# ChainSafe/Spectre

Hardware: NVIDIA H100
Metric: bn254_g1_msm_pairs_per_s (higher is better)
Workload: dtype u256 (8x32-bit Montgomery limbs, INT32 IMAD)

## Files before the change

spectre_b200/csrc/msm.cu:

```cuda
#define SPB_MSM_KERNELS 1
#include "common.cuh"
#include "msm.cuh"
#include <cub/device/device_scan.cuh>
#include <string.h>

using namespace spb;

struct SrsShard {
  int dev_index = 0;
  size_t start = 0, count = 0;
  G1Affine* g = nullptr;
  G1Affine* g_lagrange = nullptr;
};
struct spb_srs {
  uint32_t k = 0;
  size_t n = 0;
  unsigned char g2[128] = {0}, s_g2[128] = {0};
  uint32_t table_c = 0;
  std::vector<SrsShard> shards;
};


namespace spb {

typedef MsmLane Lane;
static const size_t kLanePinnedBytes = 256 * 1024;
static int get_lane(spb_ctx* ctx, int dev_index, int lane_index, Lane** out) {
  Lane& l = ctx->dev[dev_index].lanes[lane_index];
  if (!l.ready) {
    SPB_CUDA(ctx, cudaStreamCreateWithFlags(&l.stream, cudaStreamNonBlocking));
    for (int i = 0; i < 9; i++) SPB_CUDA(ctx, cudaEventCreate(&l.ev[i]));
    SPB_CUDA(ctx, cudaMallocHost(&l.pinned, kLanePinnedBytes));
    l.ready = true;
  }
  *out = &l;
  return 0;
}

void msm_release_ctx(spb_ctx* ctx) {
  for (auto& d : ctx->dev) {
    cudaSetDevice(d.device);
    for (auto& l : d.lanes) {
      if (!l.ready) continue;
      cudaStreamSynchronize(l.stream);
      for (int i = 0; i < 9; i++) cudaEventDestroy(l.ev[i]);
      cudaFreeHost(l.pinned);
      cudaStreamDestroy(l.stream);
      l = Lane();
    }
  }
}

static void* lane_slot(spb_ctx* ctx, DeviceState& d, int lane, const char* name, size_t bytes) {
  char buf[64];
  snprintf(buf, sizeof buf, "%s#%d", name, lane);
  return slot(ctx, d, buf, bytes);
}

static uint32_t choose_chunk(const DeviceState& d, uint64_t est_entries) {
  const double wave = (double)d.sm_count * 512.0;
  if (est_entries >= kLongChunkMinEntries) return kLongChunk;
  double waves = (double)est_entries / 32.0 / wave;
  if (waves < 1.0) return 32;
  double w = waves < 1.5 ? 1.0 : (double)(uint64_t)(waves + 0.5);
  uint32_t L = (uint32_t)((double)est_entries / (w * wave)) + 1;
  if (L < 24) L = 24;
  if (L > 48) L = 48;
  return L;
}

static int msm_enqueue(spb_ctx* ctx, DeviceState& d, int lane, Lane& ln, const Fr* d_scalars, const G1Affine* d_bases, uint64_t n, MsmGeom g) {
  const uint64_t nb = (uint64_t)g.BW * g.B;
  const uint64_t cap = n * g.W;
  const uint32_t Lmin = g.L == kLongChunk ? kShortChunk : g.L;
  const uint64_t Tmax = (cap + Lmin - 1) / Lmin;
  if (cap >= 0x7fffffffull) return set_error(ctx, SPB_ERR_ARG, "msm: %llu entries exceed the 31-bit sort index", (unsigned long long)cap);
  uint32_t* counts = (uint32_t*)lane_slot(ctx, d, lane, "msm_counts", (nb + 1) * 4);
  uint32_t* offsets = (uint32_t*)lane_slot(ctx, d, lane, "msm_offsets", (nb + 1) * 4);
  MsmEntry* ent = (MsmEntry*)lane_slot(ctx, d, lane, "msm_entries", (cap + 1) * sizeof(MsmEntry));
  G1Xyzz* buckets = (G1Xyzz*)lane_slot(ctx, d, lane, "msm_buckets", nb * sizeof(G1Xyzz));
  uint32_t* head_key = (uint32_t*)lane_slot(ctx, d, lane, "msm_head_key", (Tmax + 1) * 4);
  uint32_t* tail_key = (uint32_t*)lane_slot(ctx, d, lane, "msm_tail_key", (Tmax + 1) * 4);
  G1Xyzz* head = (G1Xyzz*)lane_slot(ctx, d, lane, "msm_head", (Tmax + 1) * sizeof(G1Xyzz));
  G1Xyzz* tail = (G1Xyzz*)lane_slot(ctx, d, lane, "msm_tail", (Tmax + 1) * sizeof(G1Xyzz));
  uint32_t* giant = (uint32_t*)lane_slot(ctx, d, lane, "msm_giant", (Tmax + 2) * 4);
  const uint64_t max_huge = Tmax / kHugeChain + 1;
  uint32_t* huge = (uint32_t*)lane_slot(ctx, d, lane, "msm_huge", (2 * max_huge + 2) * 4);
  G1Xyzz* huge_part = (G1Xyzz*)lane_slot(ctx, d, lane, "msm_huge_part", max_huge * kHugeBlocks * sizeof(G1Xyzz));
  const MsmTail tl = msm_tail_shape(g.c);
  const uint32_t R = 1u << tl.r_log, C = 1u << tl.c_log, per = msm_tail_partials(tl);
  const uint32_t T1 = g.B >> tl.m_log;
  const uint64_t ngroups = (uint64_t)g.BW * T1;
  G1Xyzz* grp = (G1Xyzz*)lane_slot(ctx, d, lane, "msm_groups", 2 * ngroups * sizeof(G1Xyzz));
  G1Xyzz* seg_out = (G1Xyzz*)lane_slot(ctx, d, lane, "msm_rowcol", (uint64_t)g.BW * (2 * R + C) * sizeof(G1Xyzz));
  G1Xyzz* win_out = (G1Xyzz*)lane_slot(ctx, d, lane, "msm_partials", (uint64_t)g.BW * per * sizeof(G1Xyzz));
  size_t scan_bytes = 0;
  cub::DeviceScan::ExclusiveSum(nullptr, scan_bytes, counts, offsets, (int)(nb + 1), ln.stream);
  void* scan_tmp = lane_slot(ctx, d, lane, "msm_scan_tmp", scan_bytes ? scan_bytes : 16);
  if (!counts || !offsets || !ent || !buckets || !head_key || !tail_key || !head || !tail || !giant || !huge || !huge_part || !grp || !seg_out || !win_out || !scan_tmp)
    return SPB_ERR_OOM;
  if ((size_t)g.BW * per * sizeof(G1Xyzz) + 16 > kLanePinnedBytes) return set_error(ctx, SPB_ERR_STATE, "msm: %u window partials exceed the pinned staging area", g.BW * per);

  cudaStream_t st = ln.stream;
  SPB_CUDA(ctx, cudaMemsetAsync(giant, 0, 4, st));
  SPB_CUDA(ctx, cudaMemsetAsync(huge, 0, 4, st));
  const unsigned tb = 256;
  SPB_CUDA(ctx, cudaMemsetAsync(counts, 0, (nb + 1) * 4, st));
  cudaEventRecord(ln.ev[0], st);
  msm_count_kernel<<<(unsigned)((n + tb - 1) / tb), tb, 0, st>>>(n, d_scalars, g, counts);
  cudaEventRecord(ln.ev[1], st);
  SPB_CUDA(ctx, cub::DeviceScan::ExclusiveSum(scan_tmp, scan_bytes, counts, offsets, (int)(nb + 1), st));
  SPB_CUDA(ctx, cudaMemcpyAsync(counts, offsets, (nb + 1) * 4, cudaMemcpyDeviceToDevice, st));
  cudaEventRecord(ln.ev[2], st);
  msm_scatter_kernel<<<(unsigned)((n + tb - 1) / tb), tb, 0, st>>>(n, d_scalars, g, counts, ent);
  const uint32_t* total = offsets + nb;
  cudaEventRecord(ln.ev[3], st);
  msm_accumulate_kernel<<<(unsigned)((Tmax + 127) / 128), 128, 0, st>>>(total, g, ent, d_bases, buckets, head_key, head, tail_key, tail);
  cudaEventRecord(ln.ev[4], st);
  msm_stitch_kernel<<<(unsigned)((Tmax + 127) / 128), 128, 0, st>>>(total, g.L, 24, head_key, head, tail_key, tail, buckets, giant, giant + 1);
  msm_giant_kernel<<<256, 128, 0, st>>>(total, g.L, giant, giant + 1, head_key, head, tail_key, tail, buckets, huge, huge + 2);
  msm_huge_kernel<<<kHugeBlocks, 128, 0, st>>>(huge, huge + 2, head, huge_part);
  msm_huge_finish_kernel<<<64, 128, 0, st>>>(huge, huge + 2, kHugeBlocks, huge_part, tail_key, tail, buckets);
  cudaEventRecord(ln.ev[5], st);
  G1Xyzz *rows = seg_out, *cols = seg_out + (uint64_t)g.BW * R, *wrows = seg_out + (uint64_t)g.BW * (R + C);
  msm_group_kernel<<<(unsigned)((ngroups + 127) / 128), 128, 0, st>>>(ngroups, tl.m_log, offsets, buckets, grp, grp + ngroups);
  cudaEventRecord(ln.ev[6], st);
  msm_rowcol_kernel<<<g.BW * (2 * R + C), 64, 0, st>>>(T1, tl, grp, grp + ngroups, rows, cols, wrows);
  msm_weighted_kernel<<<g.BW * (2 * tl.nbr + tl.nbc), 128, 0, st>>>(tl, rows, cols, wrows, win_out);
  cudaEventRecord(ln.ev[7], st);
  SPB_CUDA(ctx, cudaGetLastError());
  ctx->n_kernel_launches += 10;
  SPB_CUDA(ctx, cudaMemcpyAsync(ln.pinned, win_out, (size_t)g.BW * per * sizeof(G1Xyzz), cudaMemcpyDeviceToHost, st));
  SPB_CUDA(ctx, cudaMemcpyAsync((char*)ln.pinned + (size_t)g.BW * per * sizeof(G1Xyzz), total, 4, cudaMemcpyDeviceToHost, st));
  return 0;
}

static G1Xyzz msm_finish(Lane& ln, MsmGeom g, uint64_t* adds) {
  const MsmTail tl = msm_tail_shape(g.c);
  const uint32_t per = msm_tail_partials(tl);
  const G1Xyzz* P = (const G1Xyzz*)ln.pinned;
  uint32_t M; memcpy(&M, (const char*)ln.pinned + (size_t)g.BW * per * sizeof(G1Xyzz), 4);
  if (adds) *adds += (uint64_t)M + 2ull * g.BW * g.B;
  std::vector<G1Xyzz> S(g.BW);
  for (uint32_t w = 0; w < g.BW; w++) S[w] = msm_tail_finish(g, P + (size_t)w * per);
  return msm_combine_windows(S.data(), g.BW, g.c);
}

static void write_result(const G1Xyzz& r, spb_g1* out) {
  G1Affine a = xyzz_to_affine(r);
  G1Jac j = jac_from_affine(a);
  memcpy(out, &j, sizeof(G1Jac));
}

struct MsmPart {
  int dev_index;
  const Fr* d_scalars;
  const Fr* h_scalars;
  int peer_src_device;
  const G1Affine* d_bases;
  uint64_t n;
  MsmGeom g;
};

static int job_enqueue(spb_ctx* ctx, int lane, std::vector<MsmPart>& parts) {
  for (auto& p : parts) {
    if (!p.n) continue;
    DeviceState& d = ctx->dev[p.dev_index];
    SPB_CUDA(ctx, cudaSetDevice(d.device));
    Lane* ln; SPB_TRY(get_lane(ctx, p.dev_index, lane, &ln));
    p.g.L = choose_chunk(d, p.n * p.g.W);
    const Fr* ds = p.d_scalars;
    DeviceState& src = p.peer_src_device >= 0 ? ctx->dev[0] : d;
    if (&src != &d) SPB_CUDA(ctx, cudaSetDevice(src.device));
    SPB_CUDA(ctx, cudaEventRecord(src.dep_ev, src.stream));
    if (&src != &d) SPB_CUDA(ctx, cudaSetDevice(d.device));
    SPB_CUDA(ctx, cudaStreamWaitEvent(ln->stream, src.dep_ev, 0));
    SPB_CUDA(ctx, cudaEventRecord(ln->ev[8], ln->stream));
    if (p.h_scalars || p.peer_src_device >= 0) {
      Fr* buf = (Fr*)lane_slot(ctx, d, lane, "msm_scalars", p.n * sizeof(Fr));
      if (!buf) return SPB_ERR_OOM;
      if (p.h_scalars) SPB_CUDA(ctx, cudaMemcpyAsync(buf, p.h_scalars, p.n * sizeof(Fr), cudaMemcpyHostToDevice, ln->stream));
      else SPB_CUDA(ctx, cudaMemcpyPeerAsync(buf, d.device, p.d_scalars, p.peer_src_device, p.n * sizeof(Fr), ln->stream));
      ds = buf;
    }
    SPB_TRY(msm_enqueue(ctx, d, lane, *ln, ds, p.d_bases, p.n, p.g));
  }
  return 0;
}

static int job_collect(spb_ctx* ctx, int lane, const std::vector<MsmPart>& parts, spb_g1* out) {
  G1Xyzz acc = xyzz_identity();
  float worst = 0.f;
  for (auto& p : parts) {
    if (!p.n) continue;
    DeviceState& d = ctx->dev[p.dev_index];
    SPB_CUDA(ctx, cudaSetDevice(d.device));
    Lane* ln; SPB_TRY(get_lane(ctx, p.dev_index, lane, &ln));
    SPB_CUDA(ctx, cudaStreamSynchronize(ln->stream));
    float ms = 0.f;
    SPB_CUDA(ctx, cudaEventElapsedTime(&ms, ln->ev[8], ln->ev[7]));
    if (ms > worst) worst = ms;
    if (p.dev_index == 0) for (int e = 0; e < 7; e++) cudaEventElapsedTime(&ctx->msm_stage_ms[e], ln->ev[e], ln->ev[e + 1]);
    G1Xyzz r = msm_finish(*ln, p.g, &ctx->last_msm_adds);
// ... 484 lines not shown
```

spectre_b200/csrc/msm.cuh:

```cuda
#pragma once
#include <stdlib.h>
#include "curve.cuh"

namespace spb {

struct MsmGeom {
  uint32_t c;
  uint32_t W;
  uint32_t B;
  uint32_t L;
  uint32_t BW;
  uint32_t precomp;
  uint32_t tab_stride;
};

struct alignas(8) MsmEntry { uint32_t key, val; };

static const uint32_t kLongChunk = 96, kShortChunk = 32;
#ifndef SPB_LONG_CHUNK_MIN_ENTRIES
#define SPB_LONG_CHUNK_MIN_ENTRIES (1ull << 23)
#endif
static const uint64_t kLongChunkMinEntries = SPB_LONG_CHUNK_MIN_ENTRIES;
SPB_HD uint32_t msm_effective_chunk(uint32_t L, uint64_t M) { return (L == kLongChunk && M < kLongChunkMinEntries) ? kShortChunk : L; }

static const uint32_t kNoKey = 0xffffffffu;

#if defined(__CUDA_ARCH__)
SPB_D uint32_t spb_atomic_inc(uint32_t* p) { return atomicAdd(p, 1u); }
#else
inline uint32_t spb_atomic_inc(uint32_t* p) { uint32_t v = *p; *p = v + 1; return v; }
#endif

struct DigitIter {
  uint32_t limbs[8];
  uint32_t c, carry, w;
  SPB_HD void init(const Fr& canonical, uint32_t c_) {
    for (int i = 0; i < 8; i++) limbs[i] = canonical.l[i];
    c = c_; carry = 0; w = 0;
  }
  SPB_HD int32_t next() {
    uint32_t bit = w * c, word = bit >> 5, sh = bit & 31;
    uint64_t v = 0;
    if (word < 8) {
      v = limbs[word];
      if (word + 1 < 8) v |= (uint64_t)limbs[word + 1] << 32;
      v >>= sh;
    }
    uint32_t raw = (uint32_t)(v & ((1u << c) - 1)) + carry;
    w++;
    if (raw > (1u << (c - 1))) { carry = 1; return (int32_t)raw - (int32_t)(1u << c); }
    carry = 0;
    return (int32_t)raw;
  }
};

SPB_HD void msm_count_thread(uint64_t tid, uint64_t n, const Fr* scalars, MsmGeom g, uint32_t* counts) {
  if (tid >= n) return;
  Fr s = fp_from_mont(scalars[tid]);
  if (fp_is_zero(s)) return;
  DigitIter it; it.init(s, g.c);
  for (uint32_t w = 0; w < g.W; w++) {
    int32_t d = it.next();
    if (d == 0) continue;
    uint32_t mag = d < 0 ? (uint32_t)(-d) : (uint32_t)d;
    spb_atomic_inc(&counts[(g.precomp ? 0u : w * g.B) + mag - 1]);
  }
}

SPB_HD void msm_scatter_thread(uint64_t tid, uint64_t n, const Fr* scalars, MsmGeom g, uint32_t* cursor, MsmEntry* ent) {
  if (tid >= n) return;
  Fr s = fp_from_mont(scalars[tid]);
  if (fp_is_zero(s)) return;
  DigitIter it; it.init(s, g.c);
  for (uint32_t w = 0; w < g.W; w++) {
    int32_t d = it.next();
    if (d == 0) continue;
    uint32_t mag = d < 0 ? (uint32_t)(-d) : (uint32_t)d;
    uint32_t key = (g.precomp ? 0u : w * g.B) + mag - 1;
    uint32_t pos = spb_atomic_inc(&cursor[key]);
    MsmEntry e; e.key = key; e.val = ((uint32_t)tid + (g.precomp ? w * g.tab_stride : 0u)) | (d < 0 ? 0x80000000u : 0u);
    ent[pos] = e;
  }
}

SPB_HD G1Affine msm_load_point(const G1Affine* bases, uint32_t val) {
#if defined(__CUDA_ARCH__)
  const uint4* q = reinterpret_cast<const uint4*>(bases + (val & 0x7fffffffu));
  uint4 a = __ldg(q), b = __ldg(q + 1), c = __ldg(q + 2), d = __ldg(q + 3);
  G1Affine p;
  p.x.l[0] = a.x; p.x.l[1] = a.y; p.x.l[2] = a.z; p.x.l[3] = a.w; p.x.l[4] = b.x; p.x.l[5] = b.y; p.x.l[6] = b.z; p.x.l[7] = b.w;
  p.y.l[0] = c.x; p.y.l[1] = c.y; p.y.l[2] = c.z; p.y.l[3] = c.w; p.y.l[4] = d.x; p.y.l[5] = d.y; p.y.l[6] = d.z; p.y.l[7] = d.w;
#else
  G1Affine p = bases[val & 0x7fffffffu];
#endif
  if (val & 0x80000000u) p.y = fp_neg(p.y);
  return p;
}

SPB_HD MsmEntry msm_load_entry(const MsmEntry* p) {
#if defined(__CUDA_ARCH__)
  uint2 v = __ldg(reinterpret_cast<const uint2*>(p));
  MsmEntry e; e.key = v.x; e.val = v.y; return e;
#else
  return *p;
#endif
}

SPB_HD void msm_accumulate_thread(uint64_t tid, uint64_t M, MsmGeom g, const MsmEntry* ent,
                                  const G1Affine* bases, G1Xyzz* buckets, uint32_t* head_key, G1Xyzz* head,
                                  uint32_t* tail_key, G1Xyzz* tail) {
  const uint32_t L = msm_effective_chunk(g.L, M);
  uint64_t lo = tid * L;
  if (lo >= M) return;
  uint64_t hi = lo + L < M ? lo + L : M;
  uint32_t hk = kNoKey, tk = kNoKey;
  MsmEntry first = msm_load_entry(ent + lo);
  uint32_t cur = first.key;
  bool run_started_before = lo > 0 && msm_load_entry(ent + lo - 1).key == cur;
  G1Xyzz acc = xyzz_from_affine(msm_load_point(bases, first.val));
  for (uint64_t e = lo + 1; e < hi; e++) {
    MsmEntry en = msm_load_entry(ent + e);
    uint32_t k = en.key;
    G1Affine p = msm_load_point(bases, en.val);
    if (k == cur) {
      xyzz_add_mixed(acc, p);
    } else {
      if (run_started_before) { hk = cur; head[tid] = acc; }
      else buckets[cur] = acc;
      run_started_before = false;
      cur = k;
      acc = xyzz_from_affine(p);
    }
  }
  bool continues = hi < M && msm_load_entry(ent + hi).key == cur;
  if (continues) {
    if (run_started_before) { hk = cur; head[tid] = acc; }
    else { tk = cur; tail[tid] = acc; }
  } else {
    if (run_started_before) { hk = cur; head[tid] = acc; }
    else buckets[cur] = acc;
  }
  head_key[tid] = hk;
  tail_key[tid] = tk;
}

SPB_HD void msm_stitch_thread(uint64_t tid, uint64_t T, uint32_t cap, const uint32_t* head_key, const G1Xyzz* head,
                              const uint32_t* tail_key, const G1Xyzz* tail, G1Xyzz* buckets, uint32_t* giant_count,
                              uint32_t* giant_list) {
  if (tid >= T) return;
  uint32_t key = tail_key[tid];
  if (key == kNoKey) return;
  uint64_t j = tid + 1, len = 0;
  while (j < T && head_key[j] == key && len <= cap) { j++; len++; }
  if (len > cap) { uint32_t slot = spb_atomic_inc(giant_count); giant_list[slot] = (uint32_t)tid; return; }
  G1Xyzz acc = tail[tid];
  for (uint64_t q = tid + 1; q < tid + 1 + len; q++) xyzz_add(acc, head[q]);
  buckets[key] = acc;
}

struct MsmTail {
  uint32_t m_log;
  uint32_t r_log, c_log;
  uint32_t nbr, nbc;
};
inline MsmTail msm_tail_shape(uint32_t c) {
  MsmTail t; uint32_t bits = c - 1;
  t.m_log = bits < 3 ? bits : 3;
  bits -= t.m_log;
  t.c_log = bits / 2; t.r_log = bits - t.c_log;
  t.nbr = ((1u << t.r_log) + 127) / 128; t.nbc = ((1u << t.c_log) + 127) / 128;
  return t;
}
SPB_HD uint32_t msm_tail_partials(const MsmTail& t) { return 3 * t.nbr + 2 * t.nbc; }

SPB_HD void msm_group_thread(uint64_t tid, uint64_t ngroups, uint32_t m_log, const uint32_t* offsets, const G1Xyzz* buckets, G1Xyzz* s1, G1Xyzz* w1) {
  if (tid >= ngroups) return;
// ... 80 lines not shown
  for (uint32_t w = 0; w < g.W; w++) {
    int32_t d = it.next();
    const bool act = live && d != 0;
    const uint32_t mag = d < 0 ? (uint32_t)(-d) : (uint32_t)d;
    const uint32_t key = (g.precomp ? 0u : w * g.B) + mag - 1;
    const unsigned peers = msm_warp_peers(act ? key : kNoKey, lane);
    if (act && lane == (uint32_t)(__ffs(peers) - 1)) atomicAdd(&counts[key], (uint32_t)__popc(peers));
  }
}
__global__ void msm_scatter_kernel(uint64_t n, const Fr* scalars, MsmGeom g, uint32_t* cursor, MsmEntry* ent) {
  const uint64_t tid = blockIdx.x * (uint64_t)blockDim.x + threadIdx.x;
  const uint32_t lane = threadIdx.x & 31u;
  bool live = tid < n;
  Fr s = live ? fp_from_mont(scalars[tid]) : fp_zero<FrParams>();
  live = live && !fp_is_zero(s);
  DigitIter it; it.init(s, g.c);
  for (uint32_t w = 0; w < g.W; w++) {
    int32_t d = it.next();
    const bool act = live && d != 0;
    const uint32_t mag = d < 0 ? (uint32_t)(-d) : (uint32_t)d;
    const uint32_t key = (g.precomp ? 0u : w * g.B) + mag - 1;
    const unsigned peers = msm_warp_peers(act ? key : kNoKey, lane);
    const uint32_t leader = (uint32_t)(__ffs(peers) - 1);
    uint32_t base = 0;
    if (act && lane == leader) base = atomicAdd(&cursor[key], (uint32_t)__popc(peers));
    base = __shfl_sync(0xffffffffu, base, leader);
    if (act) {
      const uint32_t pos = base + (uint32_t)__popc(peers & ((1u << lane) - 1u));
      MsmEntry e; e.key = key; e.val = ((uint32_t)tid + (g.precomp ? w * g.tab_stride : 0u)) | (d < 0 ? 0x80000000u : 0u);
      ent[pos] = e;
    }
  }
}
#ifndef SPB_ACC_MINBLOCKS
#define SPB_ACC_MINBLOCKS 1
#endif
__global__ void __launch_bounds__(128, SPB_ACC_MINBLOCKS) msm_accumulate_kernel(const uint32_t* total, MsmGeom g, const MsmEntry* ent,
                                                             const G1Affine* bases, G1Xyzz* buckets, uint32_t* head_key, G1Xyzz* head,
                                                             uint32_t* tail_key, G1Xyzz* tail) {
  msm_accumulate_thread(blockIdx.x * (uint64_t)blockDim.x + threadIdx.x, *total, g, ent, bases, buckets, head_key, head, tail_key, tail);
}
__global__ void __launch_bounds__(128) msm_stitch_kernel(const uint32_t* total, uint32_t L, uint32_t cap, const uint32_t* head_key, const G1Xyzz* head,
                                                         const uint32_t* tail_key, const G1Xyzz* tail, G1Xyzz* buckets, uint32_t* giant_count, uint32_t* giant_list) {
  L = msm_effective_chunk(L, *total);
  uint64_t T = ((uint64_t)*total + L - 1) / L;
  msm_stitch_thread(blockIdx.x * (uint64_t)blockDim.x + threadIdx.x, T, cap, head_key, head, tail_key, tail, buckets, giant_count, giant_list);
}

template <int NT>
__device__ void block_sum_xyzz(G1Xyzz& v, G1Xyzz* sh) {
  const int tid = threadIdx.x;
  for (int stride = NT / 2; stride >= 1; stride >>= 1) {
    if (tid >= stride && tid < 2 * stride) sh[tid - stride] = v;
    __syncthreads();
    if (tid < stride) xyzz_add(v, sh[tid]);
    __syncthreads();
  }
}

template <int NT>
__device__ void block_sum2_xyzz(G1Xyzz& a, G1Xyzz& b, G1Xyzz* sh ) {
  const int tid = threadIdx.x;
  for (int stride = NT / 2; stride >= 1; stride >>= 1) {
    if (tid >= stride && tid < 2 * stride) { sh[2 * (tid - stride)] = a; sh[2 * (tid - stride) + 1] = b; }
    __syncthreads();
    if (tid < stride) { xyzz_add(a, sh[2 * tid]); xyzz_add(b, sh[2 * tid + 1]); }
    __syncthreads();
  }
}

static const uint32_t kHugeChain = 4096;
static const uint32_t kHugeBlocks = 1056;
__global__ void __launch_bounds__(128) msm_giant_kernel(const uint32_t* total, uint32_t L, const uint32_t* giant_count, const uint32_t* giant_list,
                                                        const uint32_t* head_key, const G1Xyzz* head, const uint32_t* tail_key, const G1Xyzz* tail,
                                                        G1Xyzz* buckets, uint32_t* huge_count, uint32_t* huge_list ) {
  __shared__ G1Xyzz sh[64];
  __shared__ uint64_t s_end;
  L = msm_effective_chunk(L, *total);
  const uint64_t T = ((uint64_t)*total + L - 1) / L;
  const uint32_t count = *giant_count;
  for (uint32_t gi = blockIdx.x; gi < count; gi += gridDim.x) {
    uint64_t t0 = giant_list[gi];
    uint32_t key = tail_key[t0];
    if (threadIdx.x == 0) {
      uint64_t lo = t0 + 1, hi = T;
      while (lo < hi) { uint64_t mid = (lo + hi) >> 1; if (head_key[mid] == key) lo = mid + 1; else hi = mid; }
      s_end = lo;
    }
    __syncthreads();
    const uint64_t end = s_end;
    if (end - (t0 + 1) > kHugeChain) {
      if (threadIdx.x == 0) { uint32_t slot = atomicAdd(huge_count, 1u); huge_list[2 * slot] = (uint32_t)t0; huge_list[2 * slot + 1] = (uint32_t)end; }
      __syncthreads();
      continue;
    }
    G1Xyzz acc = xyzz_identity();
    for (uint64_t j = t0 + 1 + threadIdx.x; j < end; j += 128) xyzz_add(acc, head[j]);
    block_sum_xyzz<128>(acc, sh);
    if (threadIdx.x == 0) { xyzz_add(acc, tail[t0]); buckets[key] = acc; }
    __syncthreads();
  }
}
__global__ void __launch_bounds__(128) msm_huge_kernel(const uint32_t* huge_count, const uint32_t* huge_list, const G1Xyzz* head, G1Xyzz* partial) {
  __shared__ G1Xyzz sh[64];
  const uint32_t count = *huge_count;
  if (!count) return;
  const uint32_t nparts = gridDim.x / count ? gridDim.x / count : 1;
  for (uint64_t work = blockIdx.x; work < (uint64_t)count * nparts; work += gridDim.x) {
    const uint32_t hi = (uint32_t)(work / nparts), part = (uint32_t)(work % nparts);
    const uint64_t t0 = huge_list[2 * hi], end = huge_list[2 * hi + 1];
    G1Xyzz acc = xyzz_identity();
// ... 117 lines not shown
  uint64_t r = 0;
  for (uint32_t b = 0; b < k; b++) r |= ((tid >> b) & 1ull) << (k - 1 - b);
  out[tid] = xyzz_to_affine(xyzz_mul_scalar(p[r], fp_from_mont(scale)));
}
#if defined(__CUDACC__) && defined(SPB_MSM_KERNELS)
__global__ void __launch_bounds__(128) ec_lift_kernel(uint64_t n, const G1Affine* in, G1Xyzz* out) {
  uint64_t i = blockIdx.x * (uint64_t)blockDim.x + threadIdx.x;
  if (i < n) out[i] = xyzz_from_affine(in[i]);
}
__global__ void __launch_bounds__(128) ec_ntt_stage_kernel(uint64_t n, uint64_t half, const Fr* tw, G1Xyzz* p) {
  ec_ntt_stage_thread(blockIdx.x * (uint64_t)blockDim.x + threadIdx.x, n, half, tw, p);
}
__global__ void __launch_bounds__(128) ec_ntt_finish_kernel(uint64_t n, uint32_t k, Fr scale, const G1Xyzz* p, G1Affine* out) {
  ec_ntt_finish_thread(blockIdx.x * (uint64_t)blockDim.x + threadIdx.x, n, k, scale, p, out);
}
__global__ void fr_powers_kernel(Fr* out, Fr base, uint64_t count) {
  uint64_t i = blockIdx.x * (uint64_t)blockDim.x + threadIdx.x;
  if (i < count) out[i] = fp_pow_u64(base, i);
}
#endif

inline G1Xyzz msm_combine_windows(const G1Xyzz* S, uint32_t BW, uint32_t c) {
  G1Xyzz acc = xyzz_identity();
  for (int w = (int)BW - 1; w >= 0; w--) {
    if (w != (int)BW - 1) for (uint32_t i = 0; i < c; i++) acc = xyzz_dbl(acc);
    xyzz_add(acc, S[w]);
  }
  return acc;
}

inline MsmGeom msm_make_geometry(uint32_t c, bool precomp, uint32_t tab_stride) {
  MsmGeom g;
  g.c = c; g.W = (255 + c - 1) / c; g.B = 1u << (c - 1); g.L = 32;
  g.precomp = precomp ? 1 : 0; g.BW = precomp ? 1 : g.W; g.tab_stride = tab_stride;
  return g;
}

inline uint32_t msm_choose_c(uint64_t n, bool precomp) {
  uint32_t best = 0; double best_cost = 0;
  for (uint32_t c = 3; c <= 22; c++) {
    uint32_t W = (255 + c - 1) / c;
    double cost = 10.0 * (double)n * W + 28.0 * (precomp ? 1.0 : (double)W) * (double)(1u << (c - 1));
    if (!best || cost < best_cost) { best = c; best_cost = cost; }
  }
  return best;
}
inline MsmGeom msm_choose_geometry(uint64_t n) { return msm_make_geometry(msm_choose_c(n, false), false, 0); }

SPB_HD void msm_precompute_thread(uint64_t tid, uint64_t count, uint32_t c, uint32_t W, G1Affine* table ) {
  if (tid >= count) return;
  G1Xyzz p = xyzz_from_affine(table[tid]);
  for (uint32_t j = 1; j < W; j++) {
    for (uint32_t i = 0; i < c; i++) p = xyzz_dbl(p);
    table[(uint64_t)j * count + tid] = xyzz_to_affine(p);
  }
}
#if defined(__CUDACC__) && defined(SPB_MSM_KERNELS)
__global__ void __launch_bounds__(128) msm_precompute_kernel(uint64_t count, uint32_t c, uint32_t W, G1Affine* table) {
  msm_precompute_thread(blockIdx.x * (uint64_t)blockDim.x + threadIdx.x, count, c, W, table);
}
#endif

}
```

spectre_b200/csrc/curve.cuh:

```cuda
#pragma once
#include "field.cuh"

namespace spb {

struct alignas(16) G1Affine { Fq x, y; };
struct alignas(16) G1Jac    { Fq x, y, z; };
struct alignas(16) G1Xyzz   { Fq x, y, zz, zzz; };

SPB_HD bool affine_is_identity(const G1Affine& p) { return fp_is_zero(p.x) && fp_is_zero(p.y); }
SPB_HD bool xyzz_is_identity(const G1Xyzz& p) { return fp_is_zero(p.zz); }
SPB_HD G1Xyzz xyzz_identity() {
  G1Xyzz r; r.x = fp_zero<FqParams>(); r.y = fp_one<FqParams>(); r.zz = fp_zero<FqParams>(); r.zzz = fp_zero<FqParams>();
  return r;
}
SPB_HD G1Xyzz xyzz_from_affine(const G1Affine& p) {
  if (affine_is_identity(p)) return xyzz_identity();
  G1Xyzz r; r.x = p.x; r.y = p.y; r.zz = fp_one<FqParams>(); r.zzz = fp_one<FqParams>();
  return r;
}
SPB_HD G1Affine affine_neg(const G1Affine& p) { G1Affine r; r.x = p.x; r.y = fp_neg(p.y); return r; }
SPB_HD G1Xyzz xyzz_neg(const G1Xyzz& p) { G1Xyzz r = p; r.y = fp_neg(p.y); return r; }

SPB_HD G1Xyzz xyzz_dbl_affine(const G1Affine& p) {
  Fq u = fp_dbl(p.y);
  Fq v = fp_sqr(u);
  Fq w = fp_mul(u, v);
  Fq s = fp_mul(p.x, v);
  Fq xx = fp_sqr(p.x);
  Fq m = fp_add(fp_dbl(xx), xx);
  G1Xyzz r;
  r.x = fp_sub(fp_sqr(m), fp_dbl(s));
  r.y = fp_mul_sub_mul(m, fp_sub(s, r.x), w, p.y);
  r.zz = v;
  r.zzz = w;
  return r;
}

SPB_HD G1Xyzz xyzz_dbl(const G1Xyzz& p) {
  if (xyzz_is_identity(p)) return p;
  Fq u = fp_dbl(p.y);
  Fq v = fp_sqr(u);
  Fq w = fp_mul(u, v);
  Fq s = fp_mul(p.x, v);
  Fq xx = fp_sqr(p.x);
  Fq m = fp_add(fp_dbl(xx), xx);
  G1Xyzz r;
  r.x = fp_sub(fp_sqr(m), fp_dbl(s));
  r.y = fp_mul_sub_mul(m, fp_sub(s, r.x), w, p.y);
  r.zz = fp_mul(v, p.zz);
  r.zzz = fp_mul(w, p.zzz);
  return r;
}

SPB_HD void xyzz_add_mixed(G1Xyzz& acc, const G1Affine& q) {
  if (affine_is_identity(q)) return;
  if (xyzz_is_identity(acc)) { acc.x = q.x; acc.y = q.y; acc.zz = fp_one<FqParams>(); acc.zzz = fp_one<FqParams>(); return; }
  Fq u2 = fp_mul(q.x, acc.zz);
  Fq s2 = fp_mul(q.y, acc.zzz);
  Fq p = fp_sub(u2, acc.x);
  Fq r = fp_sub(s2, acc.y);
  if (fp_is_zero(p)) {
    if (fp_is_zero(r)) acc = xyzz_dbl_affine(q);
    else acc = xyzz_identity();
    return;
  }
  Fq pp = fp_sqr(p);
  Fq ppp = fp_mul(p, pp);
  Fq qq = fp_mul(acc.x, pp);
  Fq x3 = fp_sub(fp_sub(fp_sqr(r), ppp), fp_dbl(qq));
  Fq y3 = fp_mul_sub_mul(r, fp_sub(qq, x3), acc.y, ppp);
  acc.x = x3;
  acc.y = y3;
  acc.zz = fp_mul(acc.zz, pp);
  acc.zzz = fp_mul(acc.zzz, ppp);
}

SPB_HD void xyzz_add(G1Xyzz& acc, const G1Xyzz& q) {
  if (xyzz_is_identity(q)) return;
  if (xyzz_is_identity(acc)) { acc = q; return; }
  Fq u1 = fp_mul(acc.x, q.zz);
  Fq u2 = fp_mul(q.x, acc.zz);
  Fq s1 = fp_mul(acc.y, q.zzz);
  Fq s2 = fp_mul(q.y, acc.zzz);
  Fq p = fp_sub(u2, u1);
  Fq r = fp_sub(s2, s1);
  if (fp_is_zero(p)) {
    if (fp_is_zero(r)) acc = xyzz_dbl(acc);
    else acc = xyzz_identity();
    return;
  }
  Fq pp = fp_sqr(p);
  Fq ppp = fp_mul(p, pp);
  Fq qq = fp_mul(u1, pp);
  Fq x3 = fp_sub(fp_sub(fp_sqr(r), ppp), fp_dbl(qq));
  Fq y3 = fp_mul_sub_mul(r, fp_sub(qq, x3), s1, ppp);
  acc.x = x3;
  acc.y = y3;
  acc.zz = fp_mul(fp_mul(acc.zz, q.zz), pp);
  acc.zzz = fp_mul(fp_mul(acc.zzz, q.zzz), ppp);
}

SPB_HD G1Affine xyzz_to_affine(const G1Xyzz& p) {
  G1Affine r;
  if (xyzz_is_identity(p)) { r.x = fp_zero<FqParams>(); r.y = fp_zero<FqParams>(); return r; }
  Fq izzz = fp_inv(p.zzz);
  Fq izz = fp_mul(fp_sqr(izzz), fp_sqr(p.zz));
  r.x = fp_mul(p.x, izz);
  r.y = fp_mul(p.y, izzz);
// ... 76 lines not shown
```

Before: 295.8 million.

## Double-buffer base point loads with cp.async and size chunks from occupancy wave

The accumulate kernel now prefetches the next affine base point into shared memory with cp.async double buffering, so the global gather overlaps the current mixed addition. Chunk length is now derived on the device from the measured occupancy wave (blocks per SM times SMs times threads), replacing the host heuristic, and is used consistently by the stitch and giant kernels. Launch bounds request 4 blocks per SM, which caps registers and may cause spills in the heavy field arithmetic. Shared memory use grows by 16KB per block.

```diff
diff --git a/spectre_b200/csrc/msm.cu b/spectre_b200/csrc/msm.cu
--- a/spectre_b200/csrc/msm.cu
+++ b/spectre_b200/csrc/msm.cu
@@ -57,16 +57,13 @@
   return slot(ctx, d, buf, bytes);
 }
 
-static uint32_t choose_chunk(const DeviceState& d, uint64_t est_entries) {
-  const double wave = (double)d.sm_count * 512.0;
-  if (est_entries >= kLongChunkMinEntries) return kLongChunk;
-  double waves = (double)est_entries / 32.0 / wave;
-  if (waves < 1.0) return 32;
-  double w = waves < 1.5 ? 1.0 : (double)(uint64_t)(waves + 0.5);
-  uint32_t L = (uint32_t)((double)est_entries / (w * wave)) + 1;
-  if (L < 24) L = 24;
-  if (L > 48) L = 48;
-  return L;
+static uint32_t choose_chunk(uint64_t est_entries) { return est_entries >= kLongChunkMinEntries ? kLongChunk : kShortChunk; }
+
+static int accumulate_wave(spb_ctx* ctx, const DeviceState& d, uint32_t* wave) {
+  int blocks = 0;
+  SPB_CUDA(ctx, cudaOccupancyMaxActiveBlocksPerMultiprocessor(&blocks, msm_accumulate_kernel, kAccThreads, 0));
+  *wave = (uint32_t)(blocks * d.sm_count) * kAccThreads;
+  return 0;
 }
 
 static int msm_enqueue(spb_ctx* ctx, DeviceState& d, int lane, Lane& ln, const Fr* d_scalars, const G1Affine* d_bases, uint64_t n, MsmGeom g) {
@@ -115,10 +112,10 @@
   msm_scatter_kernel<<<(unsigned)((n + tb - 1) / tb), tb, 0, st>>>(n, d_scalars, g, counts, ent);
   const uint32_t* total = offsets + nb;
   cudaEventRecord(ln.ev[3], st);
-  msm_accumulate_kernel<<<(unsigned)((Tmax + 127) / 128), 128, 0, st>>>(total, g, ent, d_bases, buckets, head_key, head, tail_key, tail);
+  msm_accumulate_kernel<<<(unsigned)((Tmax + kAccThreads - 1) / kAccThreads), kAccThreads, 0, st>>>(total, g, ent, d_bases, buckets, head_key, head, tail_key, tail);
   cudaEventRecord(ln.ev[4], st);
-  msm_stitch_kernel<<<(unsigned)((Tmax + 127) / 128), 128, 0, st>>>(total, g.L, 24, head_key, head, tail_key, tail, buckets, giant, giant + 1);
-  msm_giant_kernel<<<256, 128, 0, st>>>(total, g.L, giant, giant + 1, head_key, head, tail_key, tail, buckets, huge, huge + 2);
+  msm_stitch_kernel<<<(unsigned)((Tmax + 127) / 128), 128, 0, st>>>(total, g, 24, head_key, head, tail_key, tail, buckets, giant, giant + 1);
+  msm_giant_kernel<<<256, 128, 0, st>>>(total, g, giant, giant + 1, head_key, head, tail_key, tail, buckets, huge, huge + 2);
   msm_huge_kernel<<<kHugeBlocks, 128, 0, st>>>(huge, huge + 2, head, huge_part);
   msm_huge_finish_kernel<<<64, 128, 0, st>>>(huge, huge + 2, kHugeBlocks, huge_part, tail_key, tail, buckets);
   cudaEventRecord(ln.ev[5], st);
@@ -168,7 +165,8 @@
     DeviceState& d = ctx->dev[p.dev_index];
     SPB_CUDA(ctx, cudaSetDevice(d.device));
     Lane* ln; SPB_TRY(get_lane(ctx, p.dev_index, lane, &ln));
-    p.g.L = choose_chunk(d, p.n * p.g.W);
+    p.g.L = choose_chunk(p.n * p.g.W);
+    SPB_TRY(accumulate_wave(ctx, d, &p.g.wave));
     const Fr* ds = p.d_scalars;
     DeviceState& src = p.peer_src_device >= 0 ? ctx->dev[0] : d;
     if (&src != &d) SPB_CUDA(ctx, cudaSetDevice(src.device));
diff --git a/spectre_b200/csrc/msm.cuh b/spectre_b200/csrc/msm.cuh
--- a/spectre_b200/csrc/msm.cuh
+++ b/spectre_b200/csrc/msm.cuh
@@ -12,6 +12,7 @@
   uint32_t BW;
   uint32_t precomp;
   uint32_t tab_stride;
+  uint32_t wave;
 };
 
 struct alignas(8) MsmEntry { uint32_t key, val; };
@@ -22,6 +23,14 @@
 #endif
 static const uint64_t kLongChunkMinEntries = SPB_LONG_CHUNK_MIN_ENTRIES;
 SPB_HD uint32_t msm_effective_chunk(uint32_t L, uint64_t M) { return (L == kLongChunk && M < kLongChunkMinEntries) ? kShortChunk : L; }
+SPB_HD uint32_t msm_chunk_len(const MsmGeom& g, uint64_t M) {
+  const uint32_t L0 = msm_effective_chunk(g.L, M);
+  if (!g.wave) return L0;
+  uint64_t w = M / ((uint64_t)L0 * g.wave);
+  if (!w) w = 1;
+  const uint64_t L = (M + w * g.wave - 1) / (w * g.wave);
+  return L > L0 ? (uint32_t)L : L0;
+}
 
 static const uint32_t kNoKey = 0xffffffffu;
 
@@ -83,6 +92,10 @@
   }
 }
 
+SPB_HD G1Affine msm_signed_point(G1Affine p, uint32_t val) {
+  if (val & 0x80000000u) p.y = fp_neg(p.y);
+  return p;
+}
 SPB_HD G1Affine msm_load_point(const G1Affine* bases, uint32_t val) {
 #if defined(__CUDA_ARCH__)
   const uint4* q = reinterpret_cast<const uint4*>(bases + (val & 0x7fffffffu));
@@ -93,8 +106,7 @@
 #else
   G1Affine p = bases[val & 0x7fffffffu];
 #endif
-  if (val & 0x80000000u) p.y = fp_neg(p.y);
-  return p;
+  return msm_signed_point(p, val);
 }
 
 SPB_HD MsmEntry msm_load_entry(const MsmEntry* p) {
@@ -106,42 +118,50 @@
 #endif
 }
 
+struct MsmRun {
+  uint32_t cur;
+  uint32_t hk;
+  bool started_before;
+  G1Xyzz acc;
+};
+SPB_HD MsmRun msm_run_begin(const MsmEntry* ent, uint64_t lo, uint32_t first_key) {
+  MsmRun r;
+  r.cur = first_key; r.hk = kNoKey;
+  r.started_before = lo > 0 && msm_load_entry(ent + lo - 1).key == first_key;
+  r.acc = xyzz_identity();
+  return r;
+}
+SPB_HD void msm_run_step(MsmRun& r, uint64_t tid, uint32_t k, const G1Affine& p, G1Xyzz* buckets, G1Xyzz* head) {
+  if (k == r.cur) { xyzz_add_mixed(r.acc, p); return; }
+  if (r.started_before) { r.hk = r.cur; head[tid] = r.acc; }
+  else buckets[r.cur] = r.acc;
+  r.started_before = false;
+  r.cur = k;
+  r.acc = xyzz_from_affine(p);
+}
+SPB_HD void msm_run_flush(const MsmRun& r, uint64_t tid, bool continues, G1Xyzz* buckets, uint32_t* head_key, G1Xyzz* head,
+                          uint32_t* tail_key, G1Xyzz* tail) {
+  uint32_t hk = r.hk, tk = kNoKey;
+  if (r.started_before) { hk = r.cur; head[tid] = r.acc; }
+  else if (continues) { tk = r.cur; tail[tid] = r.acc; }
+  else buckets[r.cur] = r.acc;
+  head_key[tid] = hk;
+  tail_key[tid] = tk;
+}
+
 SPB_HD void msm_accumulate_thread(uint64_t tid, uint64_t M, MsmGeom g, const MsmEntry* ent,
                                   const G1Affine* bases, G1Xyzz* buckets, uint32_t* head_key, G1Xyzz* head,
                                   uint32_t* tail_key, G1Xyzz* tail) {
-  const uint32_t L = msm_effective_chunk(g.L, M);
-  uint64_t lo = tid * L;
+  const uint32_t L = msm_chunk_len(g, M);
+  const uint64_t lo = tid * L;
   if (lo >= M) return;
-  uint64_t hi = lo + L < M ? lo + L : M;
-  uint32_t hk = kNoKey, tk = kNoKey;
-  MsmEntry first = msm_load_entry(ent + lo);
-  uint32_t cur = first.key;
-  bool run_started_before = lo > 0 && msm_load_entry(ent + lo - 1).key == cur;
-  G1Xyzz acc = xyzz_from_affine(msm_load_point(bases, first.val));
-  for (uint64_t e = lo + 1; e < hi; e++) {
-    MsmEntry en = msm_load_entry(ent + e);
-    uint32_t k = en.key;
-    G1Affine p = msm_load_point(bases, en.val);
-    if (k == cur) {
-      xyzz_add_mixed(acc, p);
-    } else {
-      if (run_started_before) { hk = cur; head[tid] = acc; }
-      else buckets[cur] = acc;
-      run_started_before = false;
-      cur = k;
-      acc = xyzz_from_affine(p);
-    }
-  }
-  bool continues = hi < M && msm_load_entry(ent + hi).key == cur;
-  if (continues) {
-    if (run_started_before) { hk = cur; head[tid] = acc; }
-    else { tk = cur; tail[tid] = acc; }
-  } else {
-    if (run_started_before) { hk = cur; head[tid] = acc; }
-    else buckets[cur] = acc;
-  }
-  head_key[tid] = hk;
-  tail_key[tid] = tk;
+  const uint64_t hi = lo + L < M ? lo + L : M;
+  MsmRun r = msm_run_begin(ent, lo, msm_load_entry(ent + lo).key);
+  for (uint64_t e = lo; e < hi; e++) {
+    const MsmEntry en = msm_load_entry(ent + e);
+    msm_run_step(r, tid, en.key, msm_load_point(bases, en.val), buckets, head);
+  }
+  msm_run_flush(r, tid, hi < M && msm_load_entry(ent + hi).key == r.cur, buckets, head_key, head, tail_key, tail);
 }
 
 SPB_HD void msm_stitch_thread(uint64_t tid, uint64_t T, uint32_t cap, const uint32_t* head_key, const G1Xyzz* head,
@@ -288,17 +308,50 @@
     }
   }
 }
-#ifndef SPB_ACC_MINBLOCKS
-#define SPB_ACC_MINBLOCKS 1
-#endif
-__global__ void __launch_bounds__(128, SPB_ACC_MINBLOCKS) msm_accumulate_kernel(const uint32_t* total, MsmGeom g, const MsmEntry* ent,
-                                                             const G1Affine* bases, G1Xyzz* buckets, uint32_t* head_key, G1Xyzz* head,
-                                                             uint32_t* tail_key, G1Xyzz* tail) {
-  msm_accumulate_thread(blockIdx.x * (uint64_t)blockDim.x + threadIdx.x, *total, g, ent, bases, buckets, head_key, head, tail_key, tail);
-}
-__global__ void __launch_bounds__(128) msm_stitch_kernel(const uint32_t* total, uint32_t L, uint32_t cap, const uint32_t* head_key, const G1Xyzz* head,
+static const uint32_t kAccThreads = 128;
+__device__ __forceinline__ void cp_async16(void* dst, const void* src) {
+  asm volatile("cp.async.ca.shared.global [%0], [%1], 16;\n" :: "r"((uint32_t)__cvta_generic_to_shared(dst)), "l"(src) : "memory");
+}
+__device__ __forceinline__ void cp_async_commit() { asm volatile("cp.async.commit_group;\n" ::: "memory"); }
+__device__ __forceinline__ void cp_async_wait_prev() { asm volatile("cp.async.wait_group 1;\n" ::: "memory"); }
+
+__global__ void __launch_bounds__(kAccThreads, 4) msm_accumulate_kernel(const uint32_t* total, MsmGeom g, const MsmEntry* ent,
+                                                                     const G1Affine* bases, G1Xyzz* buckets, uint32_t* head_key, G1Xyzz* head,
+                                                                     uint32_t* tail_key, G1Xyzz* tail) {
+  __shared__ uint4 stage[2][4][kAccThreads];
+  const uint64_t M = *total, tid = blockIdx.x * (uint64_t)kAccThreads + threadIdx.x;
+  const uint32_t L = msm_chunk_len(g, M);
+  const uint64_t lo = tid * L;
+  if (lo >= M) return;
+  const uint64_t hi = lo + L < M ? lo + L : M;
+  auto fetch = [&](uint32_t s, uint32_t val) {
+    const uint4* q = reinterpret_cast<const uint4*>(bases + (val & 0x7fffffffu));
+    for (int i = 0; i < 4; i++) cp_async16(&stage[s][i][threadIdx.x], q + i);
+  };
+  MsmEntry cur = msm_load_entry(ent + lo);
+  MsmEntry next = lo + 1 < hi ? msm_load_entry(ent + lo + 1) : cur;
+  fetch(0, cur.val);
+  cp_async_commit();
+  MsmRun r = msm_run_begin(ent, lo, cur.key);
+  for (uint64_t e = lo; e < hi; e++) {
+    const uint32_t s = (uint32_t)(e - lo) & 1u;
+    if (e + 1 < hi) fetch(s ^ 1u, next.val);
+    cp_async_commit();
+    const MsmEntry after = e + 2 < hi ? msm_load_entry(ent + e + 2) : next;
+    cp_async_wait_prev();
+    G1Affine p;
+    const uint4 a = stage[s][0][threadIdx.x], b = stage[s][1][threadIdx.x], c = stage[s][2][threadIdx.x], d = stage[s][3][threadIdx.x];
+    p.x.l[0] = a.x; p.x.l[1] = a.y; p.x.l[2] = a.z; p.x.l[3] = a.w; p.x.l[4] = b.x; p.x.l[5] = b.y; p.x.l[6] = b.z; p.x.l[7] = b.w;
+    p.y.l[0] = c.x; p.y.l[1] = c.y; p.y.l[2] = c.z; p.y.l[3] = c.w; p.y.l[4] = d.x; p.y.l[5] = d.y; p.y.l[6] = d.z; p.y.l[7] = d.w;
+    msm_run_step(r, tid, cur.key, msm_signed_point(p, cur.val), buckets, head);
+    cur = next;
+    next = after;
+  }
+  msm_run_flush(r, tid, hi < M && msm_load_entry(ent + hi).key == r.cur, buckets, head_key, head, tail_key, tail);
+}
+__global__ void __launch_bounds__(128) msm_stitch_kernel(const uint32_t* total, MsmGeom g, uint32_t cap, const uint32_t* head_key, const G1Xyzz* head,
                                                          const uint32_t* tail_key, const G1Xyzz* tail, G1Xyzz* buckets, uint32_t* giant_count, uint32_t* giant_list) {
-  L = msm_effective_chunk(L, *total);
+  const uint32_t L = msm_chunk_len(g, *total);
   uint64_t T = ((uint64_t)*total + L - 1) / L;
   msm_stitch_thread(blockIdx.x * (uint64_t)blockDim.x + threadIdx.x, T, cap, head_key, head, tail_key, tail, buckets, giant_count, giant_list);
 }
@@ -327,12 +380,12 @@
 
 static const uint32_t kHugeChain = 4096;
 static const uint32_t kHugeBlocks = 1056;
-__global__ void __launch_bounds__(128) msm_giant_kernel(const uint32_t* total, uint32_t L, const uint32_t* giant_count, const uint32_t* giant_list,
+__global__ void __launch_bounds__(128) msm_giant_kernel(const uint32_t* total, MsmGeom g, const uint32_t* giant_count, const uint32_t* giant_list,
                                                         const uint32_t* head_key, const G1Xyzz* head, const uint32_t* tail_key, const G1Xyzz* tail,
                                                         G1Xyzz* buckets, uint32_t* huge_count, uint32_t* huge_list ) {
   __shared__ G1Xyzz sh[64];
   __shared__ uint64_t s_end;
-  L = msm_effective_chunk(L, *total);
+  const uint32_t L = msm_chunk_len(g, *total);
   const uint64_t T = ((uint64_t)*total + L - 1) / L;
   const uint32_t count = *giant_count;
   for (uint32_t gi = blockIdx.x; gi < count; gi += gridDim.x) {
@@ -516,7 +569,7 @@
 inline MsmGeom msm_make_geometry(uint32_t c, bool precomp, uint32_t tab_stride) {
   MsmGeom g;
   g.c = c; g.W = (255 + c - 1) / c; g.B = 1u << (c - 1); g.L = 32;
-  g.precomp = precomp ? 1 : 0; g.BW = precomp ? 1 : g.W; g.tab_stride = tab_stride;
+  g.precomp = precomp ? 1 : 0; g.BW = precomp ? 1 : g.W; g.tab_stride = tab_stride; g.wave = 0;
   return g;
 }
 
```

New measurement: 300.6 million, median of 6. +1.6%, better.

## Double-buffer base point loads via cp.async into shared memory in accumulate kernel

Applied to the files above, without the earlier changes.

The bucket accumulation kernel now prefetches the next sorted entry's affine base point into a per-thread double-buffered shared memory stage with cp.async, overlapping the global gather with the current mixed addition. Point coordinates are read from shared memory on use, and the entry stream is software-pipelined two ahead. Launch bounds change to a minimum of 4 blocks per SM and the shared memory carveout is set to fit the staging buffers. The occupancy constraint may force register spills in the heavy field arithmetic, and the shared memory reads add some latency.

```diff
diff --git a/spectre_b200/csrc/curve.cuh b/spectre_b200/csrc/curve.cuh
--- a/spectre_b200/csrc/curve.cuh
+++ b/spectre_b200/csrc/curve.cuh
@@ -52,15 +52,24 @@
   return r;
 }
 
-SPB_HD void xyzz_add_mixed(G1Xyzz& acc, const G1Affine& q) {
-  if (affine_is_identity(q)) return;
-  if (xyzz_is_identity(acc)) { acc.x = q.x; acc.y = q.y; acc.zz = fp_one<FqParams>(); acc.zzz = fp_one<FqParams>(); return; }
-  Fq u2 = fp_mul(q.x, acc.zz);
-  Fq s2 = fp_mul(q.y, acc.zzz);
+struct AffineSrc {
+  const G1Affine& p;
+  SPB_HD bool is_identity() const { return affine_is_identity(p); }
+  SPB_HD Fq x() const { return p.x; }
+  SPB_HD Fq y() const { return p.y; }
+  SPB_HD G1Affine point() const { return p; }
+};
+
+template <class Src>
+SPB_HD void xyzz_add_mixed_src(G1Xyzz& acc, const Src& q) {
+  if (q.is_identity()) return;
+  if (xyzz_is_identity(acc)) { acc.x = q.x(); acc.y = q.y(); acc.zz = fp_one<FqParams>(); acc.zzz = fp_one<FqParams>(); return; }
+  Fq u2 = fp_mul(q.x(), acc.zz);
+  Fq s2 = fp_mul(q.y(), acc.zzz);
   Fq p = fp_sub(u2, acc.x);
   Fq r = fp_sub(s2, acc.y);
   if (fp_is_zero(p)) {
-    if (fp_is_zero(r)) acc = xyzz_dbl_affine(q);
+    if (fp_is_zero(r)) acc = xyzz_dbl_affine(q.point());
     else acc = xyzz_identity();
     return;
   }
@@ -74,6 +83,7 @@
   acc.zz = fp_mul(acc.zz, pp);
   acc.zzz = fp_mul(acc.zzz, ppp);
 }
+SPB_HD void xyzz_add_mixed(G1Xyzz& acc, const G1Affine& q) { xyzz_add_mixed_src(acc, AffineSrc{q}); }
 
 SPB_HD void xyzz_add(G1Xyzz& acc, const G1Xyzz& q) {
   if (xyzz_is_identity(q)) return;
diff --git a/spectre_b200/csrc/msm.cu b/spectre_b200/csrc/msm.cu
--- a/spectre_b200/csrc/msm.cu
+++ b/spectre_b200/csrc/msm.cu
@@ -28,6 +28,10 @@
 static int get_lane(spb_ctx* ctx, int dev_index, int lane_index, Lane** out) {
   Lane& l = ctx->dev[dev_index].lanes[lane_index];
   if (!l.ready) {
+    int smem_sm = 0;
+    SPB_CUDA(ctx, cudaDeviceGetAttribute(&smem_sm, cudaDevAttrMaxSharedMemoryPerMultiprocessor, ctx->dev[dev_index].device));
+    const int need = (int)(kAccMinBlocks * (2 * 4 * kAccThreads * 16 + 1024));
+    SPB_CUDA(ctx, cudaFuncSetAttribute(msm_accumulate_kernel, cudaFuncAttributePreferredSharedMemoryCarveout, std::min(100, (need * 100 + smem_sm - 1) / smem_sm)));
     SPB_CUDA(ctx, cudaStreamCreateWithFlags(&l.stream, cudaStreamNonBlocking));
     for (int i = 0; i < 9; i++) SPB_CUDA(ctx, cudaEventCreate(&l.ev[i]));
     SPB_CUDA(ctx, cudaMallocHost(&l.pinned, kLanePinnedBytes));
@@ -115,7 +119,7 @@
   msm_scatter_kernel<<<(unsigned)((n + tb - 1) / tb), tb, 0, st>>>(n, d_scalars, g, counts, ent);
   const uint32_t* total = offsets + nb;
   cudaEventRecord(ln.ev[3], st);
-  msm_accumulate_kernel<<<(unsigned)((Tmax + 127) / 128), 128, 0, st>>>(total, g, ent, d_bases, buckets, head_key, head, tail_key, tail);
+  msm_accumulate_kernel<<<(unsigned)((Tmax + kAccThreads - 1) / kAccThreads), kAccThreads, 0, st>>>(total, g, ent, d_bases, buckets, head_key, head, tail_key, tail);
   cudaEventRecord(ln.ev[4], st);
   msm_stitch_kernel<<<(unsigned)((Tmax + 127) / 128), 128, 0, st>>>(total, g.L, 24, head_key, head, tail_key, tail, buckets, giant, giant + 1);
   msm_giant_kernel<<<256, 128, 0, st>>>(total, g.L, giant, giant + 1, head_key, head, tail_key, tail, buckets, huge, huge + 2);
diff --git a/spectre_b200/csrc/msm.cuh b/spectre_b200/csrc/msm.cuh
--- a/spectre_b200/csrc/msm.cuh
+++ b/spectre_b200/csrc/msm.cuh
@@ -83,20 +83,6 @@
   }
 }
 
-SPB_HD G1Affine msm_load_point(const G1Affine* bases, uint32_t val) {
-#if defined(__CUDA_ARCH__)
-  const uint4* q = reinterpret_cast<const uint4*>(bases + (val & 0x7fffffffu));
-  uint4 a = __ldg(q), b = __ldg(q + 1), c = __ldg(q + 2), d = __ldg(q + 3);
-  G1Affine p;
-  p.x.l[0] = a.x; p.x.l[1] = a.y; p.x.l[2] = a.z; p.x.l[3] = a.w; p.x.l[4] = b.x; p.x.l[5] = b.y; p.x.l[6] = b.z; p.x.l[7] = b.w;
-  p.y.l[0] = c.x; p.y.l[1] = c.y; p.y.l[2] = c.z; p.y.l[3] = c.w; p.y.l[4] = d.x; p.y.l[5] = d.y; p.y.l[6] = d.z; p.y.l[7] = d.w;
-#else
-  G1Affine p = bases[val & 0x7fffffffu];
-#endif
-  if (val & 0x80000000u) p.y = fp_neg(p.y);
-  return p;
-}
-
 SPB_HD MsmEntry msm_load_entry(const MsmEntry* p) {
 #if defined(__CUDA_ARCH__)
   uint2 v = __ldg(reinterpret_cast<const uint2*>(p));
@@ -106,30 +92,53 @@
 #endif
 }
 
-SPB_HD void msm_accumulate_thread(uint64_t tid, uint64_t M, MsmGeom g, const MsmEntry* ent,
-                                  const G1Affine* bases, G1Xyzz* buckets, uint32_t* head_key, G1Xyzz* head,
-                                  uint32_t* tail_key, G1Xyzz* tail) {
+struct MsmHostPoint {
+  const G1Affine* p;
+  bool neg;
+  SPB_HD bool is_identity() const { return affine_is_identity(*p); }
+  SPB_HD Fq x() const { return p->x; }
+  SPB_HD Fq y() const { return neg ? fp_neg(p->y) : p->y; }
+  SPB_HD G1Affine point() const { G1Affine r; r.x = x(); r.y = y(); return r; }
+};
+struct MsmHostFetch {
+  const G1Affine* bases;
+  SPB_HD void issue(uint32_t, uint32_t) {}
+  SPB_HD void ready(bool) {}
+  SPB_HD MsmHostPoint at(uint32_t, uint32_t val) const { return MsmHostPoint{bases + (val & 0x7fffffffu), (val & 0x80000000u) != 0}; }
+};
+
+template <class Fetch>
+SPB_HD void msm_accumulate_chunk(uint32_t tid, uint32_t M, const MsmGeom& g, const MsmEntry* ent, Fetch& f,
+                                 G1Xyzz* buckets, uint32_t* head_key, G1Xyzz* head, uint32_t* tail_key, G1Xyzz* tail) {
   const uint32_t L = msm_effective_chunk(g.L, M);
-  uint64_t lo = tid * L;
-  if (lo >= M) return;
-  uint64_t hi = lo + L < M ? lo + L : M;
+  if ((uint64_t)tid * L >= M) return;
+  const uint32_t lo = tid * L, hi = M - lo > L ? lo + L : M;
   uint32_t hk = kNoKey, tk = kNoKey;
-  MsmEntry first = msm_load_entry(ent + lo);
+  const MsmEntry first = msm_load_entry(ent + lo);
   uint32_t cur = first.key;
   bool run_started_before = lo > 0 && msm_load_entry(ent + lo - 1).key == cur;
-  G1Xyzz acc = xyzz_from_affine(msm_load_point(bases, first.val));
-  for (uint64_t e = lo + 1; e < hi; e++) {
-    MsmEntry en = msm_load_entry(ent + e);
-    uint32_t k = en.key;
-    G1Affine p = msm_load_point(bases, en.val);
-    if (k == cur) {
-      xyzz_add_mixed(acc, p);
+  f.issue(lo & 1, first.val);
+  MsmEntry e1 = lo + 1 < hi ? msm_load_entry(ent + lo + 1) : first;
+  if (lo + 1 < hi) f.issue((lo + 1) & 1, e1.val);
+  MsmEntry e2 = lo + 2 < hi ? msm_load_entry(ent + lo + 2) : e1;
+  f.ready(lo + 1 < hi);
+  G1Xyzz acc = xyzz_from_affine(f.at(lo & 1, first.val).point());
+  for (uint32_t e = lo + 1; e < hi; e++) {
+    const MsmEntry en = e1;
+    const bool more = e + 1 < hi;
+    if (more) f.issue((e + 1) & 1, e2.val);
+    e1 = e2;
+    if (e + 2 < hi) e2 = msm_load_entry(ent + e + 2);
+    f.ready(more);
+    const auto p = f.at(e & 1, en.val);
+    if (en.key == cur) {
+      xyzz_add_mixed_src(acc, p);
     } else {
       if (run_started_before) { hk = cur; head[tid] = acc; }
       else buckets[cur] = acc;
       run_started_before = false;
-      cur = k;
-      acc = xyzz_from_affine(p);
+      cur = en.key;
+      acc = xyzz_from_affine(p.point());
     }
   }
   bool continues = hi < M && msm_load_entry(ent + hi).key == cur;
@@ -142,6 +151,11 @@
   }
   head_key[tid] = hk;
   tail_key[tid] = tk;
+}
+inline void msm_accumulate_thread(uint64_t tid, uint64_t M, MsmGeom g, const MsmEntry* ent, const G1Affine* bases, G1Xyzz* buckets,
+                                  uint32_t* head_key, G1Xyzz* head, uint32_t* tail_key, G1Xyzz* tail) {
+  MsmHostFetch f{bases};
+  msm_accumulate_chunk((uint32_t)tid, (uint32_t)M, g, ent, f, buckets, head_key, head, tail_key, tail);
 }
 
 SPB_HD void msm_stitch_thread(uint64_t tid, uint64_t T, uint32_t cap, const uint32_t* head_key, const G1Xyzz* head,
@@ -288,13 +302,53 @@
     }
   }
 }
-#ifndef SPB_ACC_MINBLOCKS
-#define SPB_ACC_MINBLOCKS 1
-#endif
-__global__ void __launch_bounds__(128, SPB_ACC_MINBLOCKS) msm_accumulate_kernel(const uint32_t* total, MsmGeom g, const MsmEntry* ent,
-                                                             const G1Affine* bases, G1Xyzz* buckets, uint32_t* head_key, G1Xyzz* head,
-                                                             uint32_t* tail_key, G1Xyzz* tail) {
-  msm_accumulate_thread(blockIdx.x * (uint64_t)blockDim.x + threadIdx.x, *total, g, ent, bases, buckets, head_key, head, tail_key, tail);
+static const uint32_t kAccThreads = 128, kAccMinBlocks = 4;
+static const uint32_t kAccPartStride = kAccThreads * 16;
+struct MsmStagedPoint {
+  uint32_t s;
+  bool neg;
+  __device__ __forceinline__ uint4 part(uint32_t i) const {
+    uint4 v;
+    asm volatile("ld.shared.v4.u32 {%0, %1, %2, %3}, [%4];" : "=r"(v.x), "=r"(v.y), "=r"(v.z), "=r"(v.w) : "r"(s + i * kAccPartStride));
+    return v;
+  }
+  __device__ __forceinline__ Fq coord(uint32_t i) const {
+    const uint4 a = part(i), b = part(i + 1);
+    Fq r;
+    r.l[0] = a.x; r.l[1] = a.y; r.l[2] = a.z; r.l[3] = a.w; r.l[4] = b.x; r.l[5] = b.y; r.l[6] = b.z; r.l[7] = b.w;
+    return r;
+  }
+  __device__ __forceinline__ bool is_identity() const {
+    const uint4 a = part(0), b = part(1), c = part(2), d = part(3);
+    return ((a.x | a.y | a.z | a.w) | (b.x | b.y | b.z | b.w) | (c.x | c.y | c.z | c.w) | (d.x | d.y | d.z | d.w)) == 0;
+  }
+  __device__ __forceinline__ Fq x() const { return coord(0); }
+  __device__ __forceinline__ Fq y() const { const Fq v = coord(2); return neg ? fp_neg(v) : v; }
+  __device__ __forceinline__ G1Affine point() const { G1Affine r; r.x = x(); r.y = y(); return r; }
+};
+struct MsmStagedFetch {
+  const G1Affine* bases;
+  uint32_t s;
+  __device__ __forceinline__ void issue(uint32_t slot, uint32_t val) {
+    const char* src = reinterpret_cast<const char*>(bases + (val & 0x7fffffffu));
+    const uint32_t dst = s + slot * 4 * kAccPartStride;
+#pragma unroll
+    for (uint32_t i = 0; i < 4; i++)
+      asm volatile("cp.async.cg.shared.global [%0], [%1], 16;" :: "r"(dst + i * kAccPartStride), "l"(src + 16 * i) : "memory");
+    asm volatile("cp.async.commit_group;" ::: "memory");
+  }
+  __device__ __forceinline__ void ready(bool pending) {
+    if (pending) asm volatile("cp.async.wait_group 1;" ::: "memory");
+    else asm volatile("cp.async.wait_group 0;" ::: "memory");
+  }
+  __device__ __forceinline__ MsmStagedPoint at(uint32_t slot, uint32_t val) const { return MsmStagedPoint{s + slot * 4 * kAccPartStride, (val & 0x80000000u) != 0}; }
+};
+__global__ void __launch_bounds__(kAccThreads, kAccMinBlocks) msm_accumulate_kernel(const uint32_t* total, MsmGeom g, const MsmEntry* ent,
+                                                                                    const G1Affine* bases, G1Xyzz* buckets, uint32_t* head_key, G1Xyzz* head,
+                                                                                    uint32_t* tail_key, G1Xyzz* tail) {
+  __shared__ uint4 stage[2 * 4 * kAccThreads];
+  MsmStagedFetch f{bases, (uint32_t)__cvta_generic_to_shared(stage + threadIdx.x)};
+  msm_accumulate_chunk(blockIdx.x * kAccThreads + threadIdx.x, *total, g, ent, f, buckets, head_key, head, tail_key, tail);
 }
 __global__ void __launch_bounds__(128) msm_stitch_kernel(const uint32_t* total, uint32_t L, uint32_t cap, const uint32_t* head_key, const G1Xyzz* head,
                                                          const uint32_t* tail_key, const G1Xyzz* tail, G1Xyzz* buckets, uint32_t* giant_count, uint32_t* giant_list) {
```

New measurement: 296.1 million before, 297.2 million after, median of 6. No clear change (+0.4%).
